# google/image-compression

Measured on AMD Instinct MI355X. Metric: Mpixels/s encode (DXT1, 4096x4096 RGBA8), higher is better.
Workload: dtype int32; 1 GPU; BASELINE config c2: DXT1 encode 4096x4096 RGBA8 on 1x MI355X, bit-exact vs reference; DXT1 encode of 16 x 4096x4096 RGBA8 textures per GPU per step (one launch), device-resident; preset=c2, codec=dxt1_rgba8, src_bytes_per_pixel=4, parallelism=independent textures per GPU, texture_range per rank (no data-path collective), world_size=1, visible_gpus=1, kernel=icamd_dxt1_rgba8_kernel

## Files before the change

### image-compression_amd/csrc/dxt_kernels.hip

```cpp
#include "dxt_block.h"
#include "dxt_plan.h"
#include "ic_launch.h"
#include "ic_amd.h"

namespace icamd {

template <int COMPS, bool DXT5, bool WIDE, bool THROUGH = false, uint32_t LANES = kThreadsPerWorkgroup>
__device__ __forceinline__ void dxt_encode_one(const GridParams &P) {
  const TileCoord t = locate_tile<WIDE, 1, LANES>(P);
  if (!t.valid) return;
  uint32_t px[16];
  load_tile_block<COMPS>(P, t, px);
  const bool swap = P.swap_rb != 0;
  __shared__ uint32_t lds_px[4][LANES][4];
  BlockStashRows<LANES * 4> stash;
  stash.base = &lds_px[0][threadIdx.x][0];
  if (DXT5) {
    const bool one_pixel = (t.bcol * 4 >= P.width) && (t.brow * 4 >= P.height);
    const Out8 a = encode_dxt5_alpha_block(px, one_pixel);
    const Out8 c = encode_dxt_color_block(px, swap, true, stash);
    store_stream16(tile_dst<16>(P, t), a.lo, a.hi, c.lo, c.hi);
  } else {
    const Out8 c = encode_dxt_color_block(px, swap, false, stash);
    if (THROUGH) store_through8(tile_dst<8>(P, t), c.lo, c.hi);
    else store_stream8(tile_dst<8>(P, t), c.lo, c.hi);
  }
}

template <int COMPS, bool DXT5, bool THROUGH>
__device__ __forceinline__ void dxt_encode_two(const GridParams &P) {
  const TileCoord t = locate_tile<true, 2>(P);
  __shared__ uint32_t lds_px[4][kThreadsPerWorkgroup][4];
  BlockStash stash;
  stash.base = &lds_px[0][threadIdx.x][0];
  const bool swap = P.swap_rb != 0;
  TileCoord tr[2];
  uint32_t px[2][16];
#pragma unroll
  for (int r = 0; r < 2; ++r) {
    tr[r] = t;
    tr[r].brow0 = t.brow0 + (uint32_t)r;
    tr[r].brow = tr[r].brow0;
    tr[r].valid = t.full || (t.bcol < P.block_cols && tr[r].brow < P.block_rows);
    if (tr[r].valid) load_tile_block<COMPS>(P, tr[r], px[r]);
  }
#pragma unroll
  for (int r = 0; r < 2; ++r) {
    if (!tr[r].valid) continue;
    if (DXT5) {
      const bool one_pixel = (tr[r].bcol * 4 >= P.width) && (tr[r].brow * 4 >= P.height);
      const Out8 a = encode_dxt5_alpha_block(px[r], one_pixel);
      const Out8 c = encode_dxt_color_block(px[r], swap, true, stash);
      store_stream16(tile_dst<16>(P, tr[r]), a.lo, a.hi, c.lo, c.hi);
    } else {
      const Out8 c = encode_dxt_color_block(px[r], swap, false, stash);
      if (THROUGH) store_through8(tile_dst<8>(P, tr[r]), c.lo, c.hi);
      else store_stream8(tile_dst<8>(P, tr[r]), c.lo, c.hi);
    }
  }
}

extern "C" {

__global__ void __launch_bounds__(kThreadsPerWorkgroup) icamd_dxt1_rgb888_x2_kernel(GridParams P) { dxt_encode_two<3, false, true>(P); }

__global__ void __launch_bounds__(64) icamd_dxt1_rgba8_kernel(GridParams P) { dxt_encode_one<4, false, true, true, 64>(P); }
__global__ void __launch_bounds__(64) icamd_dxt1_rgba8_nt_kernel(GridParams P) { dxt_encode_one<4, false, true, false, 64>(P); }
__global__ void __launch_bounds__(kThreadsPerWorkgroup) icamd_dxt1_rgb888_x2_nt_kernel(GridParams P) { dxt_encode_two<3, false, false>(P); }
__global__ void __launch_bounds__(kThreadsPerWorkgroup) icamd_dxt5_rgba8_kernel(GridParams P) { dxt_encode_one<4, true, true>(P); }
__global__ void __launch_bounds__(kThreadsPerWorkgroup) icamd_dxt1_rgba8_narrow_kernel(GridParams P) { dxt_encode_one<4, false, false>(P); }
__global__ void __launch_bounds__(kThreadsPerWorkgroup) icamd_dxt1_rgb888_narrow_kernel(GridParams P) { dxt_encode_one<3, false, false>(P); }
__global__ void __launch_bounds__(kThreadsPerWorkgroup) icamd_dxt5_rgba8_narrow_kernel(GridParams P) { dxt_encode_one<4, true, false>(P); }

}

const char *dxt_kernel_name(int codec, int comps) {
  if (codec == ICAMD_DXT5) return "icamd_dxt5_rgba8_kernel";
  return comps == 4 ? "icamd_dxt1_rgba8_kernel" : "icamd_dxt1_rgb888_x2_kernel";
}

hipError_t launch_dxt(int codec, int comps, const GridParams &P, hipStream_t stream) {
  const DxtLaunchForm form = dxt_launch_form(codec, comps, P.block_cols, P.row_stride);
  if (codec == ICAMD_DXT5) {
    if (comps != 4) return hipErrorInvalidValue;
    return launch_tiled(icamd_dxt5_rgba8_kernel, icamd_dxt5_rgba8_narrow_kernel, P, stream, 8, form.wide_rows, form.wave_workgroups);
  }
  const bool through = (((uintptr_t)P.dst | P.dst_image_stride) & 7u) == 0;
  if (comps == 4)
    return launch_tiled(through ? icamd_dxt1_rgba8_kernel : icamd_dxt1_rgba8_nt_kernel, icamd_dxt1_rgba8_narrow_kernel, P, stream, 8,
                        form.wide_rows, form.wave_workgroups);
  return launch_tiled(through ? icamd_dxt1_rgb888_x2_kernel : icamd_dxt1_rgb888_x2_nt_kernel, icamd_dxt1_rgb888_narrow_kernel, P,
                      stream, 8, form.wide_rows, form.wave_workgroups);
}

}
```

### image-compression_amd/csrc/dxt_plan.h

```cpp
#ifndef ICAMD_DXT_PLAN_H_
#define ICAMD_DXT_PLAN_H_

#include <cstdint>

#include "etc2_mip_plan.h"

namespace icamd {

struct DxtLaunchForm {
  uint32_t log2_tile_cols;
  uint32_t wide_rows;
  bool wave_workgroups;
  uint32_t lanes, grid_x;
};

inline bool dxt_wave_workgroups(int codec, int comps) { return codec == ICAMD_DXT1 && comps == 4; }

inline DxtLaunchForm dxt_launch_form(int codec, int comps, uint32_t block_cols, uint32_t row_stride) {
  DxtLaunchForm f;
  f.log2_tile_cols = encode_tile_shape(block_cols, row_stride, 8u).log2_tile_cols;
  f.wide_rows = codec == ICAMD_DXT1 && comps == 3 ? 2u : 1u;
  f.wave_workgroups = f.log2_tile_cols == 8u && dxt_wave_workgroups(codec, comps);
  f.lanes = f.wave_workgroups ? 64u : 256u;
  const uint32_t cols = f.wave_workgroups ? 64u : 1u << f.log2_tile_cols;
  const uint32_t tiles = (uint32_t)(((uint64_t)block_cols + (1u << f.log2_tile_cols) - 1u) >> f.log2_tile_cols);
  f.grid_x = tiles * ((1u << f.log2_tile_cols) / cols);
  return f;
}

}
#endif
```

Baseline: 1.460 million Mpixels/s.

## Add specialized 3D-grid DXT1 RGBA8 kernel for whole, aligned textures

```diff
diff --git a/image-compression_amd/csrc/dxt_kernels.hip b/image-compression_amd/csrc/dxt_kernels.hip
--- a/image-compression_amd/csrc/dxt_kernels.hip
+++ b/image-compression_amd/csrc/dxt_kernels.hip
@@ -25,6 +25,22 @@
     if (THROUGH) store_through8(tile_dst<8>(P, t), c.lo, c.hi);
     else store_stream8(tile_dst<8>(P, t), c.lo, c.hi);
   }
+}
+
+template <bool THROUGH>
+__device__ __forceinline__ void dxt1_rgba8_fast(const uint8_t *__restrict__ src, uint8_t *__restrict__ dst, uint64_t src_image_stride,
+                                                uint64_t dst_image_stride, uint64_t src_row_pitch, uint32_t row_stride,
+                                                uint32_t dst_row_pitch, uint32_t flags) {
+  uint32_t px[16];
+  load_block_interior<4>(src + dxt_fast_src_offset(src_image_stride, src_row_pitch, blockIdx.x, blockIdx.y, blockIdx.z),
+                         threadIdx.x * 16u, row_stride, px);
+  __shared__ uint32_t lds_px[4][64][4];
+  WaveBlockStash stash;
+  stash.base = &lds_px[0][threadIdx.x][0];
+  const Out8 c = encode_dxt_color_block(px, (flags & kDxtFastSwapRb) != 0, false, stash);
+  uint8_t *out = dst + dxt_fast_dst_offset(dst_image_stride, dst_row_pitch, blockIdx.x, blockIdx.y, blockIdx.z) + threadIdx.x * 8u;
+  if (THROUGH) store_through8(out, c.lo, c.hi);
+  else store_stream8(out, c.lo, c.hi);
 }
 
 template <int COMPS, bool DXT5, bool THROUGH>
@@ -64,8 +80,18 @@
 
 __global__ void __launch_bounds__(kThreadsPerWorkgroup) icamd_dxt1_rgb888_x2_kernel(GridParams P) { dxt_encode_two<3, false, true>(P); }
 
-__global__ void __launch_bounds__(64) icamd_dxt1_rgba8_kernel(GridParams P) { dxt_encode_one<4, false, true, true, 64>(P); }
-__global__ void __launch_bounds__(64) icamd_dxt1_rgba8_nt_kernel(GridParams P) { dxt_encode_one<4, false, true, false, 64>(P); }
+__global__ void __launch_bounds__(64) icamd_dxt1_rgba8_grid_kernel(GridParams P) { dxt_encode_one<4, false, true, true, 64>(P); }
+__global__ void __launch_bounds__(64) icamd_dxt1_rgba8_grid_nt_kernel(GridParams P) { dxt_encode_one<4, false, true, false, 64>(P); }
+#define ICAMD_DXT_FAST_ARGS                                                                                                  \
+  const uint8_t *src, uint8_t *dst, uint64_t src_image_stride, uint64_t dst_image_stride, uint64_t src_row_pitch,           \
+      uint32_t row_stride, uint32_t dst_row_pitch, uint32_t flags
+__global__ void __launch_bounds__(64) icamd_dxt1_rgba8_kernel(ICAMD_DXT_FAST_ARGS) {
+  dxt1_rgba8_fast<true>(src, dst, src_image_stride, dst_image_stride, src_row_pitch, row_stride, dst_row_pitch, flags);
+}
+__global__ void __launch_bounds__(64) icamd_dxt1_rgba8_nt_kernel(ICAMD_DXT_FAST_ARGS) {
+  dxt1_rgba8_fast<false>(src, dst, src_image_stride, dst_image_stride, src_row_pitch, row_stride, dst_row_pitch, flags);
+}
+#undef ICAMD_DXT_FAST_ARGS
 __global__ void __launch_bounds__(kThreadsPerWorkgroup) icamd_dxt1_rgb888_x2_nt_kernel(GridParams P) { dxt_encode_two<3, false, false>(P); }
 __global__ void __launch_bounds__(kThreadsPerWorkgroup) icamd_dxt5_rgba8_kernel(GridParams P) { dxt_encode_one<4, true, true>(P); }
 __global__ void __launch_bounds__(kThreadsPerWorkgroup) icamd_dxt1_rgba8_narrow_kernel(GridParams P) { dxt_encode_one<4, false, false>(P); }
@@ -79,6 +105,23 @@
   return comps == 4 ? "icamd_dxt1_rgba8_kernel" : "icamd_dxt1_rgb888_x2_kernel";
 }
 
+static hipError_t launch_dxt_fast(const DxtFastPlan &fast, const GridParams &P, hipStream_t stream) {
+  if (P.n_images == 0) return hipSuccess;
+  (void)hipGetLastError();
+  for (uint32_t first = 0; first < P.n_images; first += kDxtFastMaxGridYZ) {
+    const uint32_t count = P.n_images - first < kDxtFastMaxGridYZ ? P.n_images - first : kDxtFastMaxGridYZ;
+    for (uint32_t row0 = 0; row0 < fast.grid_y; row0 += kDxtFastMaxGridYZ) {
+      const uint32_t rows = fast.grid_y - row0 < kDxtFastMaxGridYZ ? fast.grid_y - row0 : kDxtFastMaxGridYZ;
+      const DxtFastBases b = dxt_fast_bases(fast, (uint64_t)(uintptr_t)P.src, (uint64_t)(uintptr_t)P.dst, P.src_image_stride,
+                                            P.dst_image_stride, first, row0);
+      hipLaunchKernelGGL(fast.through ? icamd_dxt1_rgba8_kernel : icamd_dxt1_rgba8_nt_kernel, dim3(fast.grid_x, rows, count), dim3(64),
+                         0, stream, reinterpret_cast<const uint8_t *>((uintptr_t)b.src), reinterpret_cast<uint8_t *>((uintptr_t)b.dst),
+                         P.src_image_stride, P.dst_image_stride, fast.src_row_pitch, fast.row_stride, fast.dst_row_pitch, fast.flags);
+    }
+  }
+  return hipGetLastError();
+}
+
 hipError_t launch_dxt(int codec, int comps, const GridParams &P, hipStream_t stream) {
   const DxtLaunchForm form = dxt_launch_form(codec, comps, P.block_cols, P.row_stride);
   if (codec == ICAMD_DXT5) {
@@ -86,9 +129,12 @@
     return launch_tiled(icamd_dxt5_rgba8_kernel, icamd_dxt5_rgba8_narrow_kernel, P, stream, 8, form.wide_rows, form.wave_workgroups);
   }
   const bool through = (((uintptr_t)P.dst | P.dst_image_stride) & 7u) == 0;
+  const DxtFastPlan fast = dxt_fast_plan(codec, comps, P.height, P.width, P.block_rows, P.block_cols, P.row_stride, P.swap_rb != 0,
+                                         (uint64_t)(uintptr_t)P.dst, P.dst_image_stride);
+  if (fast.fast) return launch_dxt_fast(fast, P, stream);
   if (comps == 4)
-    return launch_tiled(through ? icamd_dxt1_rgba8_kernel : icamd_dxt1_rgba8_nt_kernel, icamd_dxt1_rgba8_narrow_kernel, P, stream, 8,
-                        form.wide_rows, form.wave_workgroups);
+    return launch_tiled(through ? icamd_dxt1_rgba8_grid_kernel : icamd_dxt1_rgba8_grid_nt_kernel, icamd_dxt1_rgba8_narrow_kernel, P,
+                        stream, 8, form.wide_rows, form.wave_workgroups);
   return launch_tiled(through ? icamd_dxt1_rgb888_x2_kernel : icamd_dxt1_rgb888_x2_nt_kernel, icamd_dxt1_rgb888_narrow_kernel, P,
                       stream, 8, form.wide_rows, form.wave_workgroups);
 }
diff --git a/image-compression_amd/csrc/dxt_plan.h b/image-compression_amd/csrc/dxt_plan.h
--- a/image-compression_amd/csrc/dxt_plan.h
+++ b/image-compression_amd/csrc/dxt_plan.h
@@ -28,5 +28,55 @@
   return f;
 }
 
+struct DxtFastPlan {
+  bool fast;
+  bool through;
+  uint32_t grid_x, grid_y;
+  uint64_t src_row_pitch;
+  uint32_t row_stride;
+  uint32_t dst_row_pitch;
+  uint32_t flags;
+};
+constexpr uint32_t kDxtFastSwapRb = 1u;
+constexpr uint32_t kDxtFastMaxGridYZ = 65535u;
+
+inline DxtFastPlan dxt_fast_plan(int codec, int comps, uint32_t height, uint32_t width, uint32_t block_rows, uint32_t block_cols,
+                                 uint32_t row_stride, bool swap_rb, uint64_t dst_addr, uint64_t dst_image_stride) {
+  DxtFastPlan p = {};
+  const bool whole = (uint64_t)block_cols * 4u == width && (uint64_t)block_rows * 4u == height;
+  const bool gather = encode_tile_shape(block_cols, row_stride, 8u).force_gather != 0;
+  p.fast = codec == ICAMD_DXT1 && comps == 4 && block_cols != 0 && block_rows != 0 && block_cols % 64u == 0 && whole && !gather &&
+           (uint64_t)block_cols * 8u < (1ull << 32);
+  if (!p.fast) return p;
+  p.through = ((dst_addr | dst_image_stride) & 7u) == 0;
+  p.grid_x = block_cols / 64u;
+  p.grid_y = block_rows;
+  p.src_row_pitch = (uint64_t)row_stride * 4u;
+  p.row_stride = row_stride;
+  p.dst_row_pitch = block_cols * 8u;
+  p.flags = swap_rb ? kDxtFastSwapRb : 0u;
+  return p;
+}
+
+struct DxtFastBases {
+  uint64_t src, dst;
+};
+inline DxtFastBases dxt_fast_bases(const DxtFastPlan &p, uint64_t src_addr, uint64_t dst_addr, uint64_t src_image_stride,
+                                   uint64_t dst_image_stride, uint32_t first_image, uint32_t tile_row0) {
+  DxtFastBases b;
+  b.src = src_addr + (uint64_t)first_image * src_image_stride + (uint64_t)tile_row0 * p.src_row_pitch;
+  b.dst = dst_addr + (uint64_t)first_image * dst_image_stride + (uint64_t)tile_row0 * p.dst_row_pitch;
+  return b;
+}
+
+ICAMD_PLAN_HD inline uint64_t dxt_fast_src_offset(uint64_t src_image_stride, uint64_t src_row_pitch, uint32_t bx, uint32_t by,
+                                                  uint32_t bz) {
+  return (uint64_t)bz * src_image_stride + (uint64_t)by * src_row_pitch + (uint64_t)bx * 1024u;
+}
+ICAMD_PLAN_HD inline uint64_t dxt_fast_dst_offset(uint64_t dst_image_stride, uint32_t dst_row_pitch, uint32_t bx, uint32_t by,
+                                                  uint32_t bz) {
+  return (uint64_t)bz * dst_image_stride + (uint64_t)by * dst_row_pitch + (uint64_t)bx * 512u;
+}
+
 }
 #endif
```

Result: no change. 1.462 million Mpixels/s (median of 4 runs) (+0.1%).
